# noamzilo/sed-crnn

Measured on AMD Instinct MI355X. Metric: mel-frames/sec training throughput (seq=256, mel=40), higher is better.
Workload: dtype f32; 1 GPU; BASELINE config 2: mono (B=128,256,40,1) per GPU, 3xConv3x3(128)+BN+ReLU+pool(1,2)+dropout0.5, BiGRU 2x128, Linear(256,1), BCEWithLogits, Adam lr 1e-3; full fit step (fwd+loss+bwd+allreduce+Adam); global_batch=128, seq_len=256, n_mels=40, parallelism=single

## Files before the change

### sed_crnn_amd/build.py

```python
import os
import subprocess
import sys
from concurrent.futures import ThreadPoolExecutor

HERE = os.path.dirname(os.path.abspath(__file__))
CSRC = os.path.join(HERE, "csrc")
OBJ = os.path.join(CSRC, "_obj")
LIB = os.path.join(HERE, "libsedcrnn.so")
SOURCES = ["api.cpp", "conv.hip", "conv_bf16.hip", "wino.hip", "conv1.hip", "bnpool.hip", "gemm.hip", "gru.hip", "misc.hip", "logmel.hip", "gcc.hip", "tdoa.hip", "doa.hip", "beam.hip", "mvdr.hip", "pcen.hip", "resample.hip", "data.hip", "detect.hip", "tune.hip", "stream.hip", "net.hip"]
FLAGS = ["--offload-arch=gfx950", "-O3", "-fPIC", "-std=c++17", "-Wall", "-Wno-unused-function"]
EXTRA_FLAGS = {"logmel.hip": ["-fno-slp-vectorize", "-Rpass-analysis=kernel-resource-usage"],
               "gcc.hip": ["-fno-slp-vectorize", "-Rpass-analysis=kernel-resource-usage"],
               "tdoa.hip": ["-fno-slp-vectorize", "-Rpass-analysis=kernel-resource-usage"],
               "doa.hip": ["-fno-slp-vectorize", "-Rpass-analysis=kernel-resource-usage"],
               "beam.hip": ["-fno-slp-vectorize", "-Rpass-analysis=kernel-resource-usage"],
               "mvdr.hip": ["-fno-slp-vectorize", "-Rpass-analysis=kernel-resource-usage"],
               "pcen.hip": ["-Rpass-analysis=kernel-resource-usage"],
               "conv.hip": ["-Rpass-analysis=kernel-resource-usage"],
               "wino.hip": ["-Rpass-analysis=kernel-resource-usage"],
               "conv_bf16.hip": ["-Rpass-analysis=kernel-resource-usage"],
               "gemm.hip": ["-Rpass-analysis=kernel-resource-usage"]}
NO_SPILL_KERNELS = {"conv.hip": ("conv3x3_mfma_fwd2_k", "conv3x3_mfma_fwd_bf16x3_k")}
NO_SCRATCH_KERNELS = {"wino.hip": ("conv3x3_wino_k",),
                      "conv_bf16.hip": ("conv3x3_bf16_eval_k", "gemm_bf16_nt_k"),
                      "logmel.hip": ("logmel_fft_k",),
                      "gcc.hip": ("gcc_phat_k",),
                      "tdoa.hip": ("tdoa_accum_k", "tdoa_finish_k"),
                      "doa.hip": ("doa_steer_k",),
                      "beam.hip": ("beam_sum_k", "beam_spans_k"),
                      "mvdr.hip": ("mvdr_cov_k", "mvdr_weights_k", "mvdr_apply_k", "mvdr_ring_cov_k", "mvdr_ring_apply_k"),
                      "pcen.hip": ("pcen_pass_k", "pcen_carry_k"),
                      "gemm.hip": ("gemm_f32_k",)}


def _hipcc():
    for c in (os.environ.get("HIPCC"), "/opt/rocm/bin/hipcc", "hipcc"):
        if c and (os.path.isabs(c) and os.path.exists(c) or not os.path.isabs(c)):
            return c
    raise RuntimeError("hipcc not found")


def _stale(target, deps):
    if not os.path.exists(target):
        return True
    t = os.path.getmtime(target)
    return any(os.path.getmtime(d) > t for d in deps)


def check_no_spill(remarks, kernels, allow_agprs=False):
    import re
    bad, seen, cur = [], set(), None
    for line in remarks.splitlines():
        m = re.search(r"remark: Function Name: (\S+)", line)
        if m:
            cur = next((k for k in kernels if k in m.group(1)), None)
            if cur:
                seen.add(cur)
            continue
        if cur:
            m = re.search(r"remark:\s+(ScratchSize \[bytes/lane\]|SGPRs Spill|VGPRs Spill|AGPRs): (\d+)", line)
            if m and int(m.group(2)) != 0 and not m.group(1).startswith("SGPRs") and not (allow_agprs and m.group(1) == "AGPRs"):
                bad.append(f"{cur}: {m.group(1)} = {m.group(2)}")
    bad += [f"{k}: no resource-usage remark found (kernel renamed? update NO_SPILL_KERNELS)" for k in kernels if k not in seen]
    return bad

# ... 53 lines not shown
```

### sed_crnn_amd/csrc/conv1.hip

```cpp
#include "common.h"

#define C1_TT 4
#define C1_MAXBLOCKS 2048

template <int CIN>
struct C1W { f32x4 w[9 * CIN]; f32x4 b; };

template <int CIN>
__device__ __forceinline__ void c1_load_w(C1W<CIN>& W, const float* __restrict__ wp, const float* __restrict__ bias,
                                          int Cout, int cg) {
#pragma unroll
    for (int tap = 0; tap < 9; ++tap)
#pragma unroll
        for (int ci = 0; ci < CIN; ++ci)
#pragma unroll
            for (int k = 0; k < 4; ++k) W.w[tap * CIN + ci][k] = wp[((size_t)tap * Cout + cg * 4 + k) * CIN + ci];
    W.b = bias ? *(const f32x4*)(bias + cg * 4) : (f32x4){0, 0, 0, 0};
}

template <int CIN>
__device__ __forceinline__ f32x4 c1_conv(const C1W<CIN>& W, const float* __restrict__ halo, int tl, int f, int F2) {
    f32x4 acc = W.b;
#pragma unroll
    for (int kh = 0; kh < 3; ++kh)
#pragma unroll
        for (int kw = 0; kw < 3; ++kw) {
            const float* hp = halo + ((tl + kw) * F2 + f + kh) * CIN;
#pragma unroll
            for (int ci = 0; ci < CIN; ++ci) acc += hp[ci] * W.w[(kh * 3 + kw) * CIN + ci];
        }
    return acc;
}

template <int CIN>
__device__ __forceinline__ void c1_conv2(const C1W<CIN>& W, const float* __restrict__ halo, int tl, int f, int F2,
                                         f32x4& v0, f32x4& v1) {
    float hv[4][3][CIN];
#pragma unroll
    for (int kw = 0; kw < 4; ++kw)
#pragma unroll
        for (int kh = 0; kh < 3; ++kh) {
            const float* hp = halo + ((tl + kw) * F2 + f + kh) * CIN;
#pragma unroll
            for (int ci = 0; ci < CIN; ++ci) hv[kw][kh][ci] = hp[ci];
        }
    v0 = W.b;
    v1 = W.b;
#pragma unroll
    for (int kh = 0; kh < 3; ++kh)
#pragma unroll
        for (int kw = 0; kw < 3; ++kw)
#pragma unroll
            for (int ci = 0; ci < CIN; ++ci) {
                v0 += hv[kw][kh][ci] * W.w[(kh * 3 + kw) * CIN + ci];
                v1 += hv[kw + 1][kh][ci] * W.w[(kh * 3 + kw) * CIN + ci];
            }
}

template <int CIN>
__device__ __forceinline__ void c1_stage(float* halo, const float* __restrict__ x, int b, int t0, int F, int T) {
    const int F2 = F + 2;
    const int n = (C1_TT + 2) * F2 * CIN;
    for (int i = threadIdx.x; i < n; i += 256) {
        int tt = i % (C1_TT + 2), ff = (i / (C1_TT + 2)) % F2, ci = i / ((C1_TT + 2) * F2);
        int t = t0 + tt - 1, f = ff - 1;
        float v = 0.f;
        if (t >= 0 && t < T && f >= 0 && f < F) v = x[(((size_t)b * CIN + ci) * F + f) * T + t];
        halo[(tt * F2 + ff) * CIN + ci] = v;
    }
}

template <int CIN, int MODE, bool P12>
__global__ __launch_bounds__(256) void conv1_fused_k(
    const float* __restrict__ x, const float* __restrict__ wp, const float* __restrict__ bias,
    const float* __restrict__ scale, const float* __restrict__ shift, const float* __restrict__ mean,
    const float* __restrict__ rstd, const float* __restrict__ sum_g, const float* __restrict__ sum_gx,
    const float* __restrict__ dout, float* __restrict__ out, float* __restrict__ partials,
    int B, int F, int T, int C, int pf, int pt, float drop_p, uint64_t seed, const uint64_t* __restrict__ seed_dev) {
    if (seed_dev) seed += seed_dev[0] * 0x9E3779B97F4A7C15ull;
    extern __shared__ __attribute__((aligned(16))) float smem[];
    if (P12) { pf = 1; pt = 2; }
    const int F2 = F + 2;
    float* halo = smem;
    const int tid = threadIdx.x;
    const int C4 = C >> 2, nslots = 256 / C4;
    const int cg = tid % C4, slot = tid / C4;
    const bool active = slot < nslots;
    const int tblocks = (T + C1_TT - 1) / C1_TT, ntiles = B * tblocks;
    const int Tp = T / pt, Fp = F / pf;
    const float inv_keep = drop_p > 0.f ? 1.f / (1.f - drop_p) : 1.f;
    const float invN = 1.f / ((float)B * (float)T * (float)F);

    C1W<CIN> W;
    if (active) c1_load_w<CIN>(W, wp, bias, C, cg);
    f32x4 sc = {0, 0, 0, 0}, sh = sc, mu = sc, rs = sc, sg = sc, sgx = sc;
    if (active && MODE >= 1) {
        sc = *(const f32x4*)(scale + cg * 4);
        sh = *(const f32x4*)(shift + cg * 4);
        if (MODE >= 2 && MODE != 4) { mu = *(const f32x4*)(mean + cg * 4); rs = *(const f32x4*)(rstd + cg * 4); }
        if (MODE == 3) { sg = *(const f32x4*)(sum_g + cg * 4) * invN; sgx = *(const f32x4*)(sum_gx + cg * 4) * invN; }
    }
    f32x4 a1 = {0, 0, 0, 0}, a2 = {0, 0, 0, 0};
    f32x4 dw[MODE == 3 ? 9 * CIN : 1];
    if (MODE == 3) {
#pragma unroll
        for (int k = 0; k < 9 * CIN; ++k) dw[k] = (f32x4){0, 0, 0, 0};
    }

    for (int tile = blockIdx.x; tile < ntiles; tile += gridDim.x) {
        const int b = tile / tblocks, t0 = (tile - b * tblocks) * C1_TT;
        __syncthreads();
        c1_stage<CIN>(halo, x, b, t0, F, T);
        __syncthreads();
        if (!active) continue;
        if (MODE == 0) {
            for (int p = slot; p < C1_TT * F; p += nslots) {
                int tl = p / F, f = p - tl * F;
                if (t0 + tl >= T) break;
                f32x4 v = c1_conv<CIN>(W, halo, tl, f, F2);
                a1 += v;
                a2 += v * v;
            }
        } else {
            const int tpn = C1_TT / pt;
            for (int op = slot; op < tpn * Fp; op += nslots) {
                int tpl = op / Fp, fp = op - tpl * Fp;
                int tp = t0 / pt + tpl;
                if (tp >= Tp) break;
                size_t oi = ((((size_t)b * Tp + tp) * Fp + fp) * C4 + cg) * 4;
                f32x4 vw[2];
                if (P12 && MODE >= 1) c1_conv2<CIN>(W, halo, tpl * 2, fp, F2, vw[0], vw[1]);
                if (MODE == 1) {
                    f32x4 m = {0, 0, 0, 0};
#pragma unroll
                    for (int df = 0; df < (P12 ? 1 : pf); ++df)
#pragma unroll
                        for (int dt = 0; dt < (P12 ? 2 : pt); ++dt) {
                            f32x4 z = (P12 ? vw[dt] : c1_conv<CIN>(W, halo, tpl * pt + dt, fp * pf + df, F2)) * sc + sh;
#pragma unroll
                            for (int k = 0; k < 4; ++k) m[k] = fmaxf(m[k], z[k]);
                        }
                    if (P12 && partials) {
                        const f32x4 z0 = vw[0] * sc + sh, z1 = vw[1] * sc + sh;
                        unsigned bt = 0;
#pragma unroll
                        for (int k = 0; k < 4; ++k) bt |= (z1[k] > z0[k] ? 1u : 0u) << k;
                        reinterpret_cast<unsigned char*>(partials)[oi >> 2] = (unsigned char)bt;
                    }
                    if (drop_p > 0.f) {
#pragma unroll
                        for (int k = 0; k < 4; ++k) m[k] *= sed_drop_mult(seed, oi + k, drop_p, inv_keep);
                    }
                    *(f32x4*)(out + oi) = m;
                } else {
                    f32x4 g = {0, 0, 0, 0};
                    if (MODE != 4) {
                        g = *(const f32x4*)(dout + oi);
                        if (drop_p > 0.f) {
#pragma unroll
                            for (int k = 0; k < 4; ++k) g[k] *= sed_drop_mult(seed, oi + k, drop_p, inv_keep);
                        }
                    }
                    f32x4 best = {-INFINITY, -INFINITY, -INFINITY, -INFINITY}, bx = {0, 0, 0, 0};
                    int bidx[4] = {0, 0, 0, 0};
                    int widx = 0;
#pragma unroll
                    for (int df = 0; df < (P12 ? 1 : pf); ++df)
#pragma unroll
                        for (int dt = 0; dt < (P12 ? 2 : pt); ++dt, ++widx) {
                            f32x4 v = P12 ? vw[dt] : c1_conv<CIN>(W, halo, tpl * pt + dt, fp * pf + df, F2);
                            f32x4 z = v * sc + sh;
#pragma unroll
                            for (int k = 0; k < 4; ++k)
                                if (z[k] > best[k]) { best[k] = z[k]; bx[k] = (v[k] - mu[k]) * rs[k]; bidx[k] = widx; }
                        }
                    if (MODE == 4) {
                        uchar4 code;
                        code.x = best[0] > 0.f ? (unsigned char)(1 + bidx[0]) : 0;
                        code.y = best[1] > 0.f ? (unsigned char)(1 + bidx[1]) : 0;
                        code.z = best[2] > 0.f ? (unsigned char)(1 + bidx[2]) : 0;
                        code.w = best[3] > 0.f ? (unsigned char)(1 + bidx[3]) : 0;
                        *(uchar4*)(reinterpret_cast<unsigned char*>(out) + oi) = code;
                        continue;
                    }
#pragma unroll
                    for (int k = 0; k < 4; ++k)
                        if (!(best[k] > 0.f)) g[k] = 0.f;
                    if (MODE == 2) {
                        a1 += g;
                        a2 += g * bx;
                    } else {
                        widx = 0;
#pragma unroll
                        for (int df = 0; df < (P12 ? 1 : pf); ++df)
#pragma unroll
                            for (int dt = 0; dt < (P12 ? 2 : pt); ++dt, ++widx) {
                                const int tl = tpl * pt + dt, f = fp * pf + df;
                                f32x4 v = P12 ? vw[dt] : c1_conv<CIN>(W, halo, tl, f, F2);
                                f32x4 o;
#pragma unroll
                                for (int k = 0; k < 4; ++k) {
                                    float xh = (v[k] - mu[k]) * rs[k];
                                    float gk = (bidx[k] == widx) ? g[k] : 0.f;
                                    o[k] = sc[k] * (gk - sg[k] - xh * sgx[k]);
                                    a2[k] += gk * xh;
                                }
                                a1 += o;
#pragma unroll
                                for (int kh = 0; kh < 3; ++kh)
#pragma unroll
                                    for (int kw = 0; kw < 3; ++kw) {
                                        const float* hp = halo + ((tl + kw) * F2 + f + kh) * CIN;
#pragma unroll
                                        for (int ci = 0; ci < CIN; ++ci) dw[(kh * 3 + kw) * CIN + ci] += hp[ci] * o;
                                    }
                            }
                    }
                }
            }
        }
    }
    if (MODE == 1 || MODE == 4) return;
    constexpr int NV = (MODE == 3) ? 2 + 9 * CIN : 2;
    constexpr int NVC = (MODE == 3) ? 5 : 2;
    float* red = smem;
#pragma unroll
    for (int v0 = 0; v0 < NV; v0 += NVC) {
        __syncthreads();
        if (active) {
#pragma unroll
            for (int j = 0; j < NVC; ++j) {
                const int v = v0 + j;
                if (v < NV) {
                    f32x4 val = (v == 0) ? a1 : ((MODE == 3 && v <= 9 * CIN) ? dw[(v - 1) < 9 * CIN ? (v - 1) : 0] : a2);
                    *(f32x4*)(red + (slot * NVC + j) * C + cg * 4) = val;
                }
            }
        }
        __syncthreads();
        const int nv = (NV - v0 < NVC) ? NV - v0 : NVC;
        for (int i = tid; i < nv * C; i += 256) {
            int j = i / C, c = i - j * C;
            float a = 0.f;
            for (int s = 0; s < nslots; ++s) a += red[(s * NVC + j) * C + c];
            partials[(size_t)blockIdx.x * NV * C + (size_t)(v0 + j) * C + c] = a;
// ... 542 lines not shown
            const double w2 = (double)wp[((size_t)(k2 / Cin) * C + co) * Cin + (k2 % Cin)];
            wg += w2 * gram[k <= k2 ? c1_gidx(k, k2, NK) : c1_gidx(k2, k, NK)];
        }
        const double s1 = gram[k];
        const double val = sc * (sv[1 + k] - sg * s1 - sgx * rs * (b * s1 + wg - mu * s1));
        const int tap = k / Cin, ci = k - tap * Cin;
        dw[((size_t)co * Cin + ci) * 9 + tap] = (float)val;
    }
    if (lane == 63) {
        const double sum_y = count * b + ws1;
        db[co] = (float)(sc * (sv[0] - count * sg - sgx * rs * (sum_y - count * mu)));
        if (dgamma && (own || (gamma && beta && gamma[co] == 0.f && beta[co] > 0.f))) dgamma[co] = (float)sgx_sum;
    }
}

static size_t c1_lds(int Cin, int F, int C, int mode) {
    size_t halo = (size_t)(C1_TT + 2) * (F + 2) * Cin * sizeof(float);
    size_t nv = mode == 3 ? 5 : 2;
    size_t red = (size_t)256 * 4 * nv * sizeof(float);
    return halo > red ? halo : red;
}

static int c1_shape_ok(int Cin, int F, int T, int C, int pool_f, int pool_t, int max_cin);
extern "C" int sed_conv1_fused_supported(int Cin, int F, int T, int C, int pool_f, int pool_t) {
    return c1_shape_ok(Cin, F, T, C, pool_f, pool_t, 2);
}
static int c1_shape_ok(int Cin, int F, int T, int C, int pool_f, int pool_t, int max_cin) {
    if (Cin < 1 || Cin > max_cin || C < 4 || F < 1 || T < 1 || C % 4 != 0 || C / 4 > 256 || (256 % (C / 4)) != 0) return 0;
    if (pool_t < 1 || pool_f < 1 || C1_TT % pool_t != 0 || T % C1_TT != 0 || F % pool_f != 0 || T % pool_t != 0) return 0;
    if (c1_lds(Cin, F, C, 3) > 150 * 1024) return 0;
    return 1;
}

extern "C" int sed_conv1_fused_rows(int B, int T) {
    long n = (long)B * ((T + C1_TT - 1) / C1_TT);
    return (int)(n < C1_MAXBLOCKS ? n : C1_MAXBLOCKS);
}

template <int MODE>
static int c1_launch(const float* x, const float* wp, const float* bias, const float* scale, const float* shift,
                     const float* mean, const float* rstd, const float* sum_g, const float* sum_gx, const float* dout,
                     float* out, float* partials, int B, int Cin, int F, int T, int C, int pf, int pt, float drop_p,
                     uint64_t seed, const uint64_t* seed_dev, hipStream_t s) {
    size_t lds = c1_lds(Cin, F, C, MODE);
    int grid = sed_conv1_fused_rows(B, T);
    const bool p12 = (pf == 1 && pt == 2);
#define C1_LAUNCH(CIN_, P12_)                                                                                          \
    do {                                                                                                               \
        if (lds > 48 * 1024)                                                                                           \
            (void)hipFuncSetAttribute((const void*)conv1_fused_k<CIN_, MODE, P12_>, hipFuncAttributeMaxDynamicSharedMemorySize, (int)lds); \
        conv1_fused_k<CIN_, MODE, P12_><<<grid, 256, lds, s>>>(x, wp, bias, scale, shift, mean, rstd, sum_g, sum_gx, dout, out, \
                                                              partials, B, F, T, C, pf, pt, drop_p, seed, seed_dev);  \
    } while (0)
    if (Cin == 1) { if (p12) C1_LAUNCH(1, true); else C1_LAUNCH(1, false); }
    else if (Cin == 2) { if (p12) C1_LAUNCH(2, true); else C1_LAUNCH(2, false); }
    else if ((MODE == 1 || MODE == 4) && p12) {
        if (Cin == 3) C1_LAUNCH(3, true);
        else C1_LAUNCH(4, true);
    } else {
        sed_set_error("conv1: %d input channels are supported by the forward pass with the (1,2) pool only", Cin);
        return SED_EUNSUPPORTED;
    }
#undef C1_LAUNCH
    return 0;
}

#define C1_CHECK(who)                                                                                             \
    SED_REQUIRE(sed_conv1_fused_supported(Cin, F, T, C, pf, pt), who ": shape Cin=%d F=%d T=%d C=%d pool=(%d,%d) is not " \
                "supported by the fused first block", Cin, F, T, C, pf, pt)

extern "C" size_t sed_conv1_stats_workspace_bytes(int B, int Cin, int T) {
    const int nk = 9 * Cin;
    if (Cin > 2) {
        const int nt = (nk + 1 + 15) / 16, np = nt * (nt + 1) / 2;
        return (size_t)C1_MM_BLOCKS * np * 256 * sizeof(float) + (size_t)(nk + nk * (nk + 1) / 2) * sizeof(double);
    }
    return (size_t)256 * (nk + nk * (nk + 1) / 2) * sizeof(float);
}

static int conv1_stats_impl(const float* x, const float* wp, const float* bias, float* stat_partials, void* workspace,
                            int B, int Cin, int F, int T, int C, double* gram_out, const Conv1BnOut& bn, void* stream);

extern "C" int sed_conv1_stats(const float* x, const float* wp, const float* bias, float* stat_partials, void* workspace,
                               int B, int Cin, int F, int T, int C, double* gram_out, void* stream) {
    return conv1_stats_impl(x, wp, bias, stat_partials, workspace, B, Cin, F, T, C, gram_out, Conv1BnOut{}, stream);
}

int sed_internal_conv1_stats_bn(const float* x, const float* wp, const float* bias, float* stat_partials, void* workspace,
                                int B, int Cin, int F, int T, int C, double* gram_out, const float* gamma, const float* beta,
                                float* running_mean, float* running_var, float momentum, float eps,
                                float* mean, float* rstd, float* scale, float* shift, void* stream) {
    SED_REQUIRE(Cin >= 1 && Cin <= 2, "conv1_stats_bn: Cin=%d (the merged finalisation exists for 1 or 2 input channels)", Cin);
    SED_REQUIRE(gamma && beta && mean && rstd && scale && shift, "conv1_stats_bn: null pointer");
    return conv1_stats_impl(x, wp, bias, stat_partials, workspace, B, Cin, F, T, C, gram_out,
                            Conv1BnOut{gamma, beta, running_mean, running_var, momentum, eps, mean, rstd, scale, shift}, stream);
}
// ... 26 lines not shown
        SED_LAUNCH_CHECK("conv1_moments");
        return 0;
    }
    int grid =(B * ((T + C1_GT - 1) / C1_GT) + C1_GR - 1) / C1_GR;
    if (grid > 256) grid = 256;
    const int nk = 9 * Cin, ng = nk + nk * (nk + 1) / 2;
    size_t lds = (size_t)C1_GR * (C1_GT + 2) * (F + 2) * Cin * sizeof(float), red = (size_t)ng * 4 * sizeof(float);
    SED_REQUIRE(lds <= 150 * 1024, "conv1_stats: F=%d Cin=%d needs %zu B of LDS", F, Cin, lds);
    if (red > lds) lds = red;
    const double count = (double)B * T * F;
    if (lds > 48 * 1024) {
        (void)hipFuncSetAttribute((const void*)conv1_gram_k<1>, hipFuncAttributeMaxDynamicSharedMemorySize, (int)lds);
        (void)hipFuncSetAttribute((const void*)conv1_gram_k<2>, hipFuncAttributeMaxDynamicSharedMemorySize, (int)lds);
    }
    if (Cin == 1) {
        conv1_gram_k<1><<<grid, 256, lds, s>>>(x, (float*)workspace, B, F, T);
        SED_LAUNCH_CHECK("conv1_gram");
        conv1_gram_finalize_k<1><<<1, 256, 0, s>>>((const float*)workspace, grid, wp, bias, count, C, stat_partials, gram_out, bn);
    } else {
        conv1_gram_k<2><<<grid, 256, lds, s>>>(x, (float*)workspace, B, F, T);
        SED_LAUNCH_CHECK("conv1_gram");
        conv1_gram_finalize_k<2><<<1, 256, 0, s>>>((const float*)workspace, grid, wp, bias, count, C, stat_partials, gram_out, bn);
    }
    SED_LAUNCH_CHECK("conv1_gram_finalize");
    return 0;
}

extern "C" int sed_conv1_bn_relu_pool_drop_fwd(const float* x, const float* wp, const float* bias, const float* scale,
                                               const float* shift, float* out, int B, int Cin, int F, int T, int C,
                                               int pf, int pt, float drop_p, uint64_t seed, const uint64_t* seed_dev,
                                               unsigned char* argmax_bits, void* stream) {
    SED_REQUIRE(x && wp && scale && shift && out, "conv1_fwd: null pointer");
    SED_REQUIRE(drop_p >= 0.f && drop_p < 1.f, "conv1_fwd: drop_p=%f out of [0,1)", drop_p);
    SED_REQUIRE(c1_shape_ok(Cin, F, T, C, pf, pt, (pf == 1 && pt == 2) ? 4 : 2), "conv1_fwd: shape Cin=%d F=%d T=%d C=%d pool=(%d,%d) is not "
                "supported by the fused first block", Cin, F, T, C, pf, pt);
    hipStream_t s = as_stream(stream);
    SedProfScope prof(SED_K_BN_FWD, s, 4.0 * B * C * (double)(T / pt) * (F / pf));
    SED_REQUIRE(!argmax_bits || (pf == 1 && pt == 2), "conv1_fwd: arg-max bits exist for the (1,2) pool only");
    SED_TRY(c1_launch<1>(x, wp, bias, scale, shift, nullptr, nullptr, nullptr, nullptr, nullptr, out, reinterpret_cast<float*>(argmax_bits), B, Cin, F, T, C, pf, pt, drop_p, seed, seed_dev, s));
    SED_LAUNCH_CHECK("conv1_fwd");
    return 0;
}

extern "C" int sed_conv1_route(const float* x, const float* wp, const float* bias, const float* scale, const float* shift,
                               unsigned char* route, int B, int Cin, int F, int T, int C, int pf, int pt, void* stream) {
    SED_REQUIRE(x && wp && scale && shift && route, "conv1_route: null pointer");
    SED_REQUIRE(c1_shape_ok(Cin, F, T, C, pf, pt, (pf == 1 && pt == 2) ? 4 : 2), "conv1_route: shape Cin=%d F=%d T=%d C=%d pool=(%d,%d) is not "
                "supported by the fused first block", Cin, F, T, C, pf, pt);
    SED_REQUIRE(pf * pt <= 254, "conv1_route: a %dx%d window does not fit the one-byte code", pf, pt);
    SED_TRY(c1_launch<4>(x, wp, bias, scale, shift, nullptr, nullptr, nullptr, nullptr, nullptr, reinterpret_cast<float*>(route), nullptr,
                         B, Cin, F, T, C, pf, pt, 0.f, 0, nullptr, as_stream(stream)));
    SED_LAUNCH_CHECK("conv1_route");
    return 0;
}

extern "C" int sed_conv1_bwd_reduce(const float* x, const float* wp, const float* bias, const float* dout,
                                    const float* scale, const float* shift, const float* mean, const float* rstd,
                                    float* partials, int B, int Cin, int F, int T, int C, int pf, int pt, float drop_p,
                                    uint64_t seed, const uint64_t* seed_dev, void* stream) {
    SED_REQUIRE(x && wp && dout && scale && shift && mean && rstd && partials, "conv1_bwd_reduce: null pointer");
    C1_CHECK("conv1_bwd_reduce");
    hipStream_t s = as_stream(stream);
    SedProfScope prof(SED_K_BN_BWD_REDUCE, s, 4.0 * B * C * (double)(T / pt) * (F / pf));
    c1_launch<2>(x, wp, bias, scale, shift, mean, rstd, nullptr, nullptr, dout, nullptr, partials, B, Cin, F, T, C, pf, pt, drop_p, seed, seed_dev, s);
    SED_LAUNCH_CHECK("conv1_bwd_reduce");
    return 0;
}

extern "C" size_t sed_conv1_bwd_apply_workspace_bytes(int B, int Cin, int T, int C) {
    return (size_t)sed_conv1_fused_rows(B, T) * (2 + 9 * Cin) * C * sizeof(float);
}

extern "C" int sed_conv1_bwd_apply_wgrad(const float* x, const float* wp, const float* bias, const float* dout,
                                         const float* scale, const float* shift, const float* mean, const float* rstd,
                                         const float* sum_g, const float* sum_gx, float* dw_oihw, float* dbias,
                                         void* workspace, int B, int Cin, int F, int T, int C, int pf, int pt,
                                         float drop_p, uint64_t seed, const uint64_t* seed_dev,
                                         const float* gamma, const float* beta, float* dgamma, void* stream) {
    SED_REQUIRE(x && wp && dout && scale && shift && mean && rstd && sum_g && sum_gx && dw_oihw && dbias && workspace,
                "conv1_bwd_apply_wgrad: null pointer");
    C1_CHECK("conv1_bwd_apply_wgrad");
    hipStream_t s = as_stream(stream);
    SedProfScope prof(SED_K_BN_BWD_APPLY, s, 4.0 * B * C * (double)(T / pt) * (F / pf));
    c1_launch<3>(x, wp, bias, scale, shift, mean, rstd, sum_g, sum_gx, dout, nullptr, (float*)workspace, B, Cin, F, T, C, pf, pt, drop_p, seed, seed_dev, s);
    SED_LAUNCH_CHECK("conv1_bwd_apply_wgrad");
    int rows = sed_conv1_fused_rows(B, T), n = (2 + 9 * Cin) * C;
    conv1_wgrad_reduce_k<<<cdiv(n, 8), 256, 0, s>>>((const float*)workspace, rows, Cin, C, dw_oihw, dbias, gamma, beta, dgamma);
    SED_LAUNCH_CHECK("conv1_wgrad_reduce");
    return 0;
}

extern "C" int sed_conv1_rgrad_supported(int Cin, int F, int T, int C, int pf, int pt) {
    return pf == 1 && pt == 2 && c1_shape_ok(Cin, F, T, C, pf, pt, 4);
}
// ... 67 lines not shown
```

### sed_crnn_amd/csrc/gru.hip

```cpp
#include "common.h"

static inline int gru_bt(int H, int B) {
    int bt = B >= 512 ? 4 : (B >= 256 ? 2 : 1);
    if (H >= 128 && bt > 2) bt = 2;
    return bt;
}

__global__ void gru_pack_whh_t_k(const float* __restrict__ w0, const float* __restrict__ w1,
                                 float* __restrict__ wt, int H) {
    int i = blockIdx.x * blockDim.x + threadIdx.x;
    int n = 3 * H * H;
    if (i >= 2 * n) return;
    int dir = i / n, e = i - dir * n;
    int g = e / H, k = e - g * H;
    const float* w = dir ? w1 : w0;
    wt[(size_t)dir * n + (size_t)k * 3 * H + g] = w[e];
}

constexpr int gru_nt(int hreg) { return hreg > 0 ? ((3 * hreg + 63) / 64) * 64 : 1024; }

__device__ __forceinline__ float gru_dot4(float w0, float w1, float w2, float w3, const f32x4& h) {
    return fmaf(w3, h[3], fmaf(w2, h[2], fmaf(w0, h[0], w1 * h[1])));
}

template <int HREG, int GRU_BT, int HTOT = HREG, int HLDS = 0>
__global__ __launch_bounds__(gru_nt(HTOT)) void gru_seq_fwd_k(
    const float* __restrict__ gi, const float* __restrict__ wt, const float* __restrict__ bhh0,
    const float* __restrict__ bhh1, float* __restrict__ out, float* __restrict__ saved, int B, int T, int H) {
    extern __shared__ __attribute__((aligned(16))) float smem[];
    float* h_s = smem;
    float* gh_s = smem + GRU_BT * H;
    float* w_l = smem + GRU_BT * 4 * H;
    const int g = threadIdx.x;
    const int dir = blockIdx.y, b0 = blockIdx.x * GRU_BT;
    const int H3 = 3 * H;
    const float* wtd = wt + (size_t)dir * H3 * H;
    const float* bhh = dir ? bhh1 : bhh0;
    const bool row = g < H3;
    const bool gate = g < H;
    constexpr bool HYB = HTOT != HREG && HREG > 0;

    float wreg[HREG > 0 ? HREG : 1];
    if (HREG > 0 && row) {
#pragma unroll
        for (int k = 0; k < HREG; ++k) wreg[k] = wtd[(size_t)k * H3 + g];
    }
    if (HYB && row) {
        for (int j = 0; j < HLDS; ++j) w_l[j * H3 + g] = wtd[(size_t)(HREG + j) * H3 + g];
    }
    const float bias = row ? bhh[g] : 0.f;
    for (int i = g; i < GRU_BT * H; i += blockDim.x) h_s[i] = 0.f;
    __syncthreads();

    float gr[GRU_BT], gz[GRU_BT], gn[GRU_BT], nr[GRU_BT], nz[GRU_BT], nn[GRU_BT], mr[GRU_BT], mz[GRU_BT], mn[GRU_BT];
    auto fetch_gi = [&](int s, float* a, float* bq, float* c) {
        const int tt = dir ? (T - 1 - s) : s;
#pragma unroll
        for (int b = 0; b < GRU_BT; ++b) {
            int bg = b0 + b;
            if (gate && bg < B && s < T) {
                const float* p = gi + (((size_t)bg * T + tt) * 2 + dir) * H3;
                a[b] = p[g]; bq[b] = p[H + g]; c[b] = p[2 * H + g];
            } else { a[b] = bq[b] = c[b] = 0.f; }
        }
    };
    fetch_gi(0, gr, gz, gn);
    fetch_gi(1, nr, nz, nn);
    for (int s = 0; s < T; ++s) {
        const int tt = dir ? (T - 1 - s) : s;
        fetch_gi(s + 2, mr, mz, mn);
        if (row) {
            float acc[GRU_BT];
#pragma unroll
            for (int b = 0; b < GRU_BT; ++b) acc[b] = bias;
            if (HREG > 0) {
#pragma unroll
                for (int k = 0; k < HREG; k += 4) {
#pragma unroll
                    for (int b = 0; b < GRU_BT; ++b) {
                        f32x4 hv = *(const f32x4*)(h_s + b * H + k);
                        acc[b] += gru_dot4(wreg[k], wreg[k + 1], wreg[k + 2], wreg[k + 3], hv);
                    }
                }
            }
// ... 229 lines not shown
    else if (v.bt == 2) KERNEL<HR, 2><<<grid, nt, lds, s>>>(__VA_ARGS__);                     \
    else KERNEL<HR, 4><<<grid, nt, lds, s>>>(__VA_ARGS__)
#define GRU_DISPATCH(KERNEL, ...)                                                             \
    if (v.hlds > 0) {                                                                         \
        KERNEL<GRU_HRX, 1, 256, GRU_HL><<<grid, nt, lds + (size_t)GRU_HL * 768 * sizeof(float), s>>>(__VA_ARGS__); \
    } else switch (v.hreg) {                                                                  \
        case 8: GRU_BT3(8, KERNEL, __VA_ARGS__); break;                                       \
        case 16: GRU_BT3(16, KERNEL, __VA_ARGS__); break;                                     \
        case 32: GRU_BT3(32, KERNEL, __VA_ARGS__); break;                                     \
        case 64: GRU_BT3(64, KERNEL, __VA_ARGS__); break;                                     \
        case 128:                                                                             \
            if (v.bt == 1) KERNEL<128, 1><<<grid, nt, lds, s>>>(__VA_ARGS__);                 \
            else KERNEL<128, 2><<<grid, nt, lds, s>>>(__VA_ARGS__);                           \
            break;                                                                            \
        default: GRU_BT3(0, KERNEL, __VA_ARGS__); break;                                      \
    }

static int gru_pack_whh(const float* const* whh, float* wt, int H, hipStream_t s) {
    int n = 2 * 3 * H * H;
    gru_pack_whh_t_k<<<cdiv(n, 256), 256, 0, s>>>(whh[0], whh[1], wt, H);
    SED_LAUNCH_CHECK("gru_pack_whh_t");
    return 0;
}

int sed_internal_gru_seq_fwd_packed(const float* gi, const float* wt, const float* const* bhh, float* out,
                                    float* saved, int B, int T, int H, void* stream) {
    SED_REQUIRE(gi && wt && bhh && out && bhh[0] && bhh[1], "gru_seq_fwd: null pointer");
    SED_REQUIRE(B > 0 && T > 0 && H > 0 && H % 4 == 0 && 3 * H <= 1024, "gru_seq_fwd: H=%d must be a multiple of 4 and <= 341", H);
    hipStream_t s = as_stream(stream);
    const GruVariant v = gru_variant(H, B, GRU_HR_FWD);
    dim3 grid(cdiv(B, v.bt), 2);
    int nt = gru_threads(H);
    size_t lds = (size_t)v.bt * 4 * H * sizeof(float);
    SedProfScope prof(SED_K_GRU_FWD, s, 2.0 * 2 * B * (double)T * 3 * H * H);
    if (v.hlds > 0)
        (void)hipFuncSetAttribute((const void*)gru_seq_fwd_k<GRU_HR_FWD, 1, 256, GRU_HL>, hipFuncAttributeMaxDynamicSharedMemorySize, 160 * 1024);
#define GRU_HRX GRU_HR_FWD
    GRU_DISPATCH(gru_seq_fwd_k, gi, wt, bhh[0], bhh[1], out, saved, B, T, H);
#undef GRU_HRX
    SED_LAUNCH_CHECK("gru_seq_fwd");
    return 0;
}

extern "C" int sed_gru_seq_fwd(const float* gi, const float* const* whh, const float* const* bhh, float* out,
                               float* saved, void* workspace, int B, int T, int H, void* stream) {
    SED_REQUIRE(gi && whh && bhh && out && workspace && whh[0] && whh[1] && bhh[0] && bhh[1], "gru_seq_fwd: null pointer");
    SED_REQUIRE(B > 0 && T > 0 && H > 0 && H % 4 == 0 && 3 * H <= 1024, "gru_seq_fwd: H=%d must be a multiple of 4 and <= 341", H);
    SED_TRY(gru_pack_whh(whh, (float*)workspace, H, as_stream(stream)));
    return sed_internal_gru_seq_fwd_packed(gi, (const float*)workspace, bhh, out, saved, B, T, H, stream);
}

extern "C" size_t sed_gru_seq_bwd_workspace_bytes(int B, int H) { return (size_t)cdiv(B, gru_bt(H, B)) * 2 * 4 * H * sizeof(float); }

int sed_internal_gru_seq_bwd_partials(const float* dout, const float* saved, const float* const* whh, float* dgi,
                                      float* dgh, float* bpart, int B, int T, int H, void* stream) {
    SED_REQUIRE(dout && saved && whh && whh[0] && whh[1] && dgi && dgh, "gru_seq_bwd: null pointer");
    SED_REQUIRE(B > 0 && T > 0 && H > 0 && H % 4 == 0 && 3 * H <= 1024, "gru_seq_bwd: H=%d must be a multiple of 4 and <= 341", H);
    hipStream_t s = as_stream(stream);
    const GruVariant v = gru_variant(H, B, GRU_HR);
    dim3 grid(cdiv(B, v.bt), 2);
    int nt = gru_threads(H);
    size_t lds = (size_t)v.bt * 6 * H * sizeof(float);
    SedProfScope prof(SED_K_GRU_BWD, s, 2.0 * 2 * B * (double)T * 3 * H * H);
    if (v.hlds > 0)
        (void)hipFuncSetAttribute((const void*)gru_seq_bwd_k<GRU_HR, 1, 256, GRU_HL>, hipFuncAttributeMaxDynamicSharedMemorySize, 160 * 1024);
#define GRU_HRX GRU_HR
// ... 25 lines not shown
```

Baseline: 6.025 million mel-frames/s.

## Warp-specialize GRU forward with LDS ring prefetch and strength-reduce conv1 indexing

The GRU forward kernel, when all recurrent weights fit in registers, now splits waves into gate, load and row roles. Loader waves prefetch input-gate values two steps ahead into a three-slot LDS ring, so global loads stay off the recurrent critical path. The fused first conv kernel replaces per-iteration divisions and 64-bit index math with incremental pointer and offset updates, and uses 32-bit dropout hashing unless the tensor is very large. It also adds occupancy hints via launch bounds and a no-spill build check. The cost is extra LDS for the ring and some added complexity in synchronisation and role dispatch.

```diff
diff --git a/sed_crnn_amd/build.py b/sed_crnn_amd/build.py
--- a/sed_crnn_amd/build.py
+++ b/sed_crnn_amd/build.py
@@ -16,6 +16,7 @@
                "beam.hip": ["-fno-slp-vectorize", "-Rpass-analysis=kernel-resource-usage"],
                "mvdr.hip": ["-fno-slp-vectorize", "-Rpass-analysis=kernel-resource-usage"],
                "pcen.hip": ["-Rpass-analysis=kernel-resource-usage"],
+               "conv1.hip": ["-Rpass-analysis=kernel-resource-usage"],
                "conv.hip": ["-Rpass-analysis=kernel-resource-usage"],
                "wino.hip": ["-Rpass-analysis=kernel-resource-usage"],
                "conv_bf16.hip": ["-Rpass-analysis=kernel-resource-usage"],
@@ -30,7 +31,8 @@
                       "beam.hip": ("beam_sum_k", "beam_spans_k"),
                       "mvdr.hip": ("mvdr_cov_k", "mvdr_weights_k", "mvdr_apply_k", "mvdr_ring_cov_k", "mvdr_ring_apply_k"),
                       "pcen.hip": ("pcen_pass_k", "pcen_carry_k"),
-                      "gemm.hip": ("gemm_f32_k",)}
+                      "gemm.hip": ("gemm_f32_k",),
+                      "conv1.hip": ("conv1_fused_k",)}
 
 
 def _hipcc():
diff --git a/sed_crnn_amd/csrc/conv1.hip b/sed_crnn_amd/csrc/conv1.hip
--- a/sed_crnn_amd/csrc/conv1.hip
+++ b/sed_crnn_amd/csrc/conv1.hip
@@ -19,13 +19,13 @@
 }
 
 template <int CIN>
-__device__ __forceinline__ f32x4 c1_conv(const C1W<CIN>& W, const float* __restrict__ halo, int tl, int f, int F2) {
+__device__ __forceinline__ f32x4 c1_conv(const C1W<CIN>& W, const float* __restrict__ hb, int F2) {
     f32x4 acc = W.b;
 #pragma unroll
     for (int kh = 0; kh < 3; ++kh)
 #pragma unroll
         for (int kw = 0; kw < 3; ++kw) {
-            const float* hp = halo + ((tl + kw) * F2 + f + kh) * CIN;
+            const float* hp = hb + (kw * F2 + kh) * CIN;
 #pragma unroll
             for (int ci = 0; ci < CIN; ++ci) acc += hp[ci] * W.w[(kh * 3 + kw) * CIN + ci];
         }
@@ -33,14 +33,13 @@
 }
 
 template <int CIN>
-__device__ __forceinline__ void c1_conv2(const C1W<CIN>& W, const float* __restrict__ halo, int tl, int f, int F2,
-                                         f32x4& v0, f32x4& v1) {
+__device__ __forceinline__ void c1_conv2(const C1W<CIN>& W, const float* __restrict__ hb, int F2, f32x4& v0, f32x4& v1) {
     float hv[4][3][CIN];
 #pragma unroll
     for (int kw = 0; kw < 4; ++kw)
 #pragma unroll
         for (int kh = 0; kh < 3; ++kh) {
-            const float* hp = halo + ((tl + kw) * F2 + f + kh) * CIN;
+            const float* hp = hb + (kw * F2 + kh) * CIN;
 #pragma unroll
             for (int ci = 0; ci < CIN; ++ci) hv[kw][kh][ci] = hp[ci];
         }
@@ -70,8 +69,14 @@
     }
 }
 
-template <int CIN, int MODE, bool P12>
-__global__ __launch_bounds__(256) void conv1_fused_k(
+constexpr int c1_waves(int cin, int mode, bool p12) {
+    if (mode == 1 || mode == 4) return cin == 1 ? 5 : (cin == 2 ? ((mode == 1 && p12) ? 3 : 4) : 2);
+    if (mode == 2) return cin == 1 ? 4 : (cin == 2 ? 3 : 2);
+    return cin <= 2 ? 2 : 1;
+}
+
+template <int CIN, int MODE, bool P12, bool IDX64 = false>
+__global__ __launch_bounds__(256, c1_waves(CIN, MODE, P12)) void conv1_fused_k(
     const float* __restrict__ x, const float* __restrict__ wp, const float* __restrict__ bias,
     const float* __restrict__ scale, const float* __restrict__ shift, const float* __restrict__ mean,
     const float* __restrict__ rstd, const float* __restrict__ sum_g, const float* __restrict__ sum_gx,
@@ -107,36 +112,60 @@
         for (int k = 0; k < 9 * CIN; ++k) dw[k] = (f32x4){0, 0, 0, 0};
     }
 
-    for (int tile = blockIdx.x; tile < ntiles; tile += gridDim.x) {
-        const int b = tile / tblocks, t0 = (tile - b * tblocks) * C1_TT;
+    const int pos_w = (MODE == 0) ? F : Fp;
+    const int row_h = (MODE == 0) ? F2 * CIN : pt * F2 * CIN;
+    const int pos_h = (MODE == 0) ? CIN : pf * CIN;
+    const int q0 = nslots / pos_w, dfp = nslots - q0 * pos_w;
+    const int tpl0 = slot / pos_w, fp0 = slot - tpl0 * pos_w;
+    const int dhb = q0 * row_h + dfp * pos_h, whb = row_h - pos_w * pos_h;
+    const unsigned doff = (unsigned)nslots * C4 * 4;
+    const int qb = gridDim.x / tblocks, qt = gridDim.x - qb * tblocks;
+    int b = blockIdx.x / tblocks, tb = blockIdx.x - b * tblocks;
+
+    for (int tile = blockIdx.x; tile < ntiles; tile += gridDim.x, b += qb, tb += qt) {
+        if (tb >= tblocks) { tb -= tblocks; ++b; }
+        const int t0 = tb * C1_TT;
         __syncthreads();
         c1_stage<CIN>(halo, x, b, t0, F, T);
         __syncthreads();
         if (!active) continue;
         if (MODE == 0) {
+            int tl = tpl0, f = fp0;
+            const float* hb = halo + tpl0 * row_h + fp0 * pos_h;
             for (int p = slot; p < C1_TT * F; p += nslots) {
-                int tl = p / F, f = p - tl * F;
                 if (t0 + tl >= T) break;
-                f32x4 v = c1_conv<CIN>(W, halo, tl, f, F2);
+                f32x4 v = c1_conv<CIN>(W, hb, F2);
                 a1 += v;
                 a2 += v * v;
+                tl += q0; f += dfp; hb += dhb;
+                if (f >= F) { f -= F; ++tl; hb += whb; }
             }
         } else {
             const int tpn = C1_TT / pt;
-            for (int op = slot; op < tpn * Fp; op += nslots) {
-                int tpl = op / Fp, fp = op - tpl * Fp;
-                int tp = t0 / pt + tpl;
-                if (tp >= Tp) break;
-                size_t oi = ((((size_t)b * Tp + tp) * Fp + fp) * C4 + cg) * 4;
+            const int tp0 = t0 / pt;
+            const size_t tbase = ((size_t)b * Tp + tp0) * Fp * C;
+            const uint32_t tb_lo = (uint32_t)tbase;
+            auto keep_mult = [&](unsigned offk) {
+                return sed_drop_mult(seed, IDX64 ? (uint64_t)tbase + offk : (uint64_t)(uint32_t)(tb_lo + offk), drop_p, inv_keep);
+            };
+            int tpl = tpl0, fp = fp0;
+            const float* hb = halo + tpl0 * row_h + fp0 * pos_h;
+            unsigned off = (unsigned)(slot * C4 + cg) * 4;
+            for (int op = slot; op < tpn * Fp; op += nslots, off += doff) {
+                if (tp0 + tpl >= Tp) break;
+                const float* hw = hb;
+                tpl += q0; fp += dfp; hb += dhb;
+                if (fp >= Fp) { fp -= Fp; ++tpl; hb += whb; }
+                const unsigned boff = off * 4u;
                 f32x4 vw[2];
-                if (P12 && MODE >= 1) c1_conv2<CIN>(W, halo, tpl * 2, fp, F2, vw[0], vw[1]);
+                if (P12 && MODE >= 1) c1_conv2<CIN>(W, hw, F2, vw[0], vw[1]);
                 if (MODE == 1) {
                     f32x4 m = {0, 0, 0, 0};
 #pragma unroll
                     for (int df = 0; df < (P12 ? 1 : pf); ++df)
 #pragma unroll
                         for (int dt = 0; dt < (P12 ? 2 : pt); ++dt) {
-                            f32x4 z = (P12 ? vw[dt] : c1_conv<CIN>(W, halo, tpl * pt + dt, fp * pf + df, F2)) * sc + sh;
+                            f32x4 z = (P12 ? vw[dt] : c1_conv<CIN>(W, hw + (dt * F2 + df) * CIN, F2)) * sc + sh;
 #pragma unroll
                             for (int k = 0; k < 4; ++k) m[k] = fmaxf(m[k], z[k]);
                         }
@@ -145,20 +174,22 @@
                         unsigned bt = 0;
 #pragma unroll
                         for (int k = 0; k < 4; ++k) bt |= (z1[k] > z0[k] ? 1u : 0u) << k;
-                        reinterpret_cast<unsigned char*>(partials)[oi >> 2] = (unsigned char)bt;
+                        (reinterpret_cast<unsigned char*>(partials) + (tbase >> 2))[off >> 2] = (unsigned char)bt;
                     }
                     if (drop_p > 0.f) {
 #pragma unroll
-                        for (int k = 0; k < 4; ++k) m[k] *= sed_drop_mult(seed, oi + k, drop_p, inv_keep);
+                        for (int k = 0; k < 4; ++k)
+                            m[k] *= keep_mult(off + k);
                     }
-                    *(f32x4*)(out + oi) = m;
+                    *(f32x4*)((char*)(out + tbase) + boff) = m;
                 } else {
                     f32x4 g = {0, 0, 0, 0};
                     if (MODE != 4) {
-                        g = *(const f32x4*)(dout + oi);
+                        g = *(const f32x4*)((const char*)(dout + tbase) + boff);
                         if (drop_p > 0.f) {
 #pragma unroll
-                            for (int k = 0; k < 4; ++k) g[k] *= sed_drop_mult(seed, oi + k, drop_p, inv_keep);
+                            for (int k = 0; k < 4; ++k)
+                                g[k] *= keep_mult(off + k);
                         }
                     }
                     f32x4 best = {-INFINITY, -INFINITY, -INFINITY, -INFINITY}, bx = {0, 0, 0, 0};
@@ -168,7 +199,7 @@
                     for (int df = 0; df < (P12 ? 1 : pf); ++df)
 #pragma unroll
                         for (int dt = 0; dt < (P12 ? 2 : pt); ++dt, ++widx) {
-                            f32x4 v = P12 ? vw[dt] : c1_conv<CIN>(W, halo, tpl * pt + dt, fp * pf + df, F2);
+                            f32x4 v = P12 ? vw[dt] : c1_conv<CIN>(W, hw + (dt * F2 + df) * CIN, F2);
                             f32x4 z = v * sc + sh;
 #pragma unroll
                             for (int k = 0; k < 4; ++k)
@@ -180,7 +211,7 @@
                         code.y = best[1] > 0.f ? (unsigned char)(1 + bidx[1]) : 0;
                         code.z = best[2] > 0.f ? (unsigned char)(1 + bidx[2]) : 0;
                         code.w = best[3] > 0.f ? (unsigned char)(1 + bidx[3]) : 0;
-                        *(uchar4*)(reinterpret_cast<unsigned char*>(out) + oi) = code;
+                        *(uchar4*)(reinterpret_cast<unsigned char*>(out) + tbase + off) = code;
                         continue;
                     }
 #pragma unroll
@@ -195,8 +226,8 @@
                         for (int df = 0; df < (P12 ? 1 : pf); ++df)
 #pragma unroll
                             for (int dt = 0; dt < (P12 ? 2 : pt); ++dt, ++widx) {
-                                const int tl = tpl * pt + dt, f = fp * pf + df;
-                                f32x4 v = P12 ? vw[dt] : c1_conv<CIN>(W, halo, tl, f, F2);
+                                const float* he = hw + (dt * F2 + df) * CIN;
+                                f32x4 v = P12 ? vw[dt] : c1_conv<CIN>(W, he, F2);
                                 f32x4 o;
 #pragma unroll
                                 for (int k = 0; k < 4; ++k) {
@@ -210,7 +241,7 @@
                                 for (int kh = 0; kh < 3; ++kh)
 #pragma unroll
                                     for (int kw = 0; kw < 3; ++kw) {
-                                        const float* hp = halo + ((tl + kw) * F2 + f + kh) * CIN;
+                                        const float* hp = he + (kw * F2 + kh) * CIN;
 #pragma unroll
                                         for (int ci = 0; ci < CIN; ++ci) dw[(kh * 3 + kw) * CIN + ci] += hp[ci] * o;
                                     }
@@ -819,6 +850,11 @@
     return 1;
 }
 
+static int c1_pass_shape_ok(int Cin, int F, int T, int C, int pool_f, int pool_t, int max_cin) {
+    if (T < 1 || pool_t < 1 || T % pool_t != 0) return 0;
+    return c1_shape_ok(Cin, F, (T + C1_TT - 1) / C1_TT * C1_TT, C, pool_f, pool_t, max_cin);
+}
+
 extern "C" int sed_conv1_fused_rows(int B, int T) {
     long n = (long)B * ((T + C1_TT - 1) / C1_TT);
     return (int)(n < C1_MAXBLOCKS ? n : C1_MAXBLOCKS);
@@ -832,12 +868,17 @@
     size_t lds = c1_lds(Cin, F, C, MODE);
     int grid = sed_conv1_fused_rows(B, T);
     const bool p12 = (pf == 1 && pt == 2);
+    const bool idx64 = MODE != 4 && drop_p > 0.f && (size_t)B * (T / pt) * (F / pf) * C > 0xFFFFFFFFull;
+#define C1_LAUNCH_(CIN_, P12_, I64_)                                                                                   \
+    do {                                                                                                               \
+        if (lds > 48 * 1024)                                                                                           \
+            (void)hipFuncSetAttribute((const void*)conv1_fused_k<CIN_, MODE, P12_, I64_>, hipFuncAttributeMaxDynamicSharedMemorySize, (int)lds); \
+        conv1_fused_k<CIN_, MODE, P12_, I64_><<<grid, 256, lds, s>>>(x, wp, bias, scale, shift, mean, rstd, sum_g, sum_gx, dout, out, \
+                                                                    partials, B, F, T, C, pf, pt, drop_p, seed, seed_dev); \
+    } while (0)
 #define C1_LAUNCH(CIN_, P12_)                                                                                          \
     do {                                                                                                               \
-        if (lds > 48 * 1024)                                                                                           \
-            (void)hipFuncSetAttribute((const void*)conv1_fused_k<CIN_, MODE, P12_>, hipFuncAttributeMaxDynamicSharedMemorySize, (int)lds); \
-        conv1_fused_k<CIN_, MODE, P12_><<<grid, 256, lds, s>>>(x, wp, bias, scale, shift, mean, rstd, sum_g, sum_gx, dout, out, \
-                                                              partials, B, F, T, C, pf, pt, drop_p, seed, seed_dev);  \
+        if (MODE != 4 && idx64) C1_LAUNCH_(CIN_, P12_, (MODE != 4)); else C1_LAUNCH_(CIN_, P12_, false);               \
     } while (0)
     if (Cin == 1) { if (p12) C1_LAUNCH(1, true); else C1_LAUNCH(1, false); }
     else if (Cin == 2) { if (p12) C1_LAUNCH(2, true); else C1_LAUNCH(2, false); }
@@ -849,6 +890,7 @@
         return SED_EUNSUPPORTED;
     }
 #undef C1_LAUNCH
+#undef C1_LAUNCH_
     return 0;
 }
 
@@ -941,7 +983,7 @@
                                                unsigned char* argmax_bits, void* stream) {
     SED_REQUIRE(x && wp && scale && shift && out, "conv1_fwd: null pointer");
     SED_REQUIRE(drop_p >= 0.f && drop_p < 1.f, "conv1_fwd: drop_p=%f out of [0,1)", drop_p);
-    SED_REQUIRE(c1_shape_ok(Cin, F, T, C, pf, pt, (pf == 1 && pt == 2) ? 4 : 2), "conv1_fwd: shape Cin=%d F=%d T=%d C=%d pool=(%d,%d) is not "
+    SED_REQUIRE(c1_pass_shape_ok(Cin, F, T, C, pf, pt, (pf == 1 && pt == 2) ? 4 : 2), "conv1_fwd: shape Cin=%d F=%d T=%d C=%d pool=(%d,%d) is not "
                 "supported by the fused first block", Cin, F, T, C, pf, pt);
     hipStream_t s = as_stream(stream);
     SedProfScope prof(SED_K_BN_FWD, s, 4.0 * B * C * (double)(T / pt) * (F / pf));
@@ -954,7 +996,7 @@
 extern "C" int sed_conv1_route(const float* x, const float* wp, const float* bias, const float* scale, const float* shift,
                                unsigned char* route, int B, int Cin, int F, int T, int C, int pf, int pt, void* stream) {
     SED_REQUIRE(x && wp && scale && shift && route, "conv1_route: null pointer");
-    SED_REQUIRE(c1_shape_ok(Cin, F, T, C, pf, pt, (pf == 1 && pt == 2) ? 4 : 2), "conv1_route: shape Cin=%d F=%d T=%d C=%d pool=(%d,%d) is not "
+    SED_REQUIRE(c1_pass_shape_ok(Cin, F, T, C, pf, pt, (pf == 1 && pt == 2) ? 4 : 2), "conv1_route: shape Cin=%d F=%d T=%d C=%d pool=(%d,%d) is not "
                 "supported by the fused first block", Cin, F, T, C, pf, pt);
     SED_REQUIRE(pf * pt <= 254, "conv1_route: a %dx%d window does not fit the one-byte code", pf, pt);
     SED_TRY(c1_launch<4>(x, wp, bias, scale, shift, nullptr, nullptr, nullptr, nullptr, nullptr, reinterpret_cast<float*>(route), nullptr,
@@ -968,7 +1010,8 @@
                                     float* partials, int B, int Cin, int F, int T, int C, int pf, int pt, float drop_p,
                                     uint64_t seed, const uint64_t* seed_dev, void* stream) {
     SED_REQUIRE(x && wp && dout && scale && shift && mean && rstd && partials, "conv1_bwd_reduce: null pointer");
-    C1_CHECK("conv1_bwd_reduce");
+    SED_REQUIRE(c1_pass_shape_ok(Cin, F, T, C, pf, pt, 2), "conv1_bwd_reduce: shape Cin=%d F=%d T=%d C=%d pool=(%d,%d) is not "
+                "supported by the fused first block", Cin, F, T, C, pf, pt);
     hipStream_t s = as_stream(stream);
     SedProfScope prof(SED_K_BN_BWD_REDUCE, s, 4.0 * B * C * (double)(T / pt) * (F / pf));
     c1_launch<2>(x, wp, bias, scale, shift, mean, rstd, nullptr, nullptr, dout, nullptr, partials, B, Cin, F, T, C, pf, pt, drop_p, seed, seed_dev, s);
diff --git a/sed_crnn_amd/csrc/gru.hip b/sed_crnn_amd/csrc/gru.hip
--- a/sed_crnn_amd/csrc/gru.hip
+++ b/sed_crnn_amd/csrc/gru.hip
@@ -23,6 +23,102 @@
     return fmaf(w3, h[3], fmaf(w2, h[2], fmaf(w0, h[0], w1 * h[1])));
 }
 
+enum { GRU_GATE = 0, GRU_LOAD = 1, GRU_ROW = 2, GRU_ALL = 3 };
+
+template <int HREG, int GRU_BT, int ROLE>
+__device__ __forceinline__ void gru_fwd_ring(const float* __restrict__ gi, float* __restrict__ out, float* __restrict__ saved,
+                                             float* h_s, float* gh_s, float* ring, const float (&wreg)[HREG], const float bias,
+                                             const int g, const int li, const int dir, const int b0, const int B, const int T, const int H) {
+    constexpr bool GATES = ROLE == GRU_GATE || ROLE == GRU_ALL, LOADS = ROLE == GRU_LOAD || ROLE == GRU_ALL;
+    const int H3 = 3 * H;
+    const bool row = g < H3, gate = g < H;
+    const bool lane = li < H;
+    const int lic = lane ? li : 0;
+    float xa[GRU_BT][3], xb[GRU_BT][3];
+    auto issue = [&](int s, float (*q)[3]) {
+        const int sc = s < T ? s : T - 1;
+        const int tt = dir ? (T - 1 - sc) : sc;
+#pragma unroll
+        for (int b = 0; b < GRU_BT; ++b) {
+            const int bg = b0 + b < B ? b0 + b : B - 1;
+            const float* p = gi + (((size_t)bg * T + tt) * 2 + dir) * H3 + lic;
+            q[b][0] = p[0]; q[b][1] = p[H]; q[b][2] = p[2 * H];
+        }
+    };
+    auto commit = [&](float (*q)[3], int slot) {
+        float* r = ring + slot * (GRU_BT * H3);
+#pragma unroll
+        for (int b = 0; b < GRU_BT; ++b) {
+            const bool in = b0 + b < B;
+            const float v0 = in ? q[b][0] : 0.f, v1 = in ? q[b][1] : 0.f, v2 = in ? q[b][2] : 0.f;
+            if (lane) { r[b * H3 + li] = v0; r[b * H3 + H + li] = v1; r[b * H3 + 2 * H + li] = v2; }
+        }
+    };
+    int rd = 0;
+    auto step = [&](int s, float (*nw)[3], float (*ld)[3]) {
+        const int tt = dir ? (T - 1 - s) : s;
+        if (LOADS) issue(s + 2, nw);
+        if (row) {
+            float acc[GRU_BT];
+#pragma unroll
+            for (int b = 0; b < GRU_BT; ++b) acc[b] = bias;
+#pragma unroll
+            for (int k = 0; k < HREG; k += 4) {
+#pragma unroll
+                for (int b = 0; b < GRU_BT; ++b) {
+                    f32x4 hv = *(const f32x4*)(h_s + b * H + k);
+                    acc[b] += gru_dot4(wreg[k], wreg[k + 1], wreg[k + 2], wreg[k + 3], hv);
+                }
+            }
+#pragma unroll
+            for (int b = 0; b < GRU_BT; ++b) gh_s[b * H3 + g] = acc[b];
+        }
+        __syncthreads();
+        if (GATES && gate) {
+            const float* rg = ring + rd * (GRU_BT * H3);
+            float gr[GRU_BT], gz[GRU_BT], gn[GRU_BT];
+#pragma unroll
+            for (int b = 0; b < GRU_BT; ++b) {
+                int bg = b0 + b;
+                gr[b] = rg[b * H3 + g]; gz[b] = rg[b * H3 + H + g]; gn[b] = rg[b * H3 + 2 * H + g];
+                float ghr = gh_s[b * H3 + g], ghz = gh_s[b * H3 + H + g], ghn = gh_s[b * H3 + 2 * H + g];
+                float hp = h_s[b * H + g];
+                float r = __fdividef(1.f, 1.f + __expf(-(gr[b] + ghr)));
+                float z = __fdividef(1.f, 1.f + __expf(-(gz[b] + ghz)));
+                float a = gn[b] + r * ghn;
+                float e2 = __expf(-2.f * fabsf(a));
+                float n = copysignf(__fdividef(1.f - e2, 1.f + e2), a);
+                float hn = (1.f - z) * n + z * hp;
+                h_s[b * H + g] = hn;
+                if (bg < B) {
+                    out[((size_t)bg * T + tt) * 2 * H + dir * H + g] = hn;
+                    if (saved) {
+                        float* sp = saved + ((((size_t)bg * T + tt) * 2 + dir) * 5) * H + g;
+                        sp[0] = r; sp[H] = z; sp[2 * H] = n; sp[3 * H] = ghn; sp[4 * H] = hp;
+                    }
+                }
+            }
+        }
+        rd = rd == 2 ? 0 : rd + 1;
+        if (LOADS) commit(ld, rd);
+        __syncthreads();
+    };
+    if (LOADS) { issue(0, xa); issue(1, xb); commit(xa, 0); }
+    __syncthreads();
+    int s = 0;
+    for (; s + 1 < T; s += 2) {
+        step(s, xa, xb);
+        step(s + 1, xb, xa);
+    }
+    if (s < T) step(s, xa, xb);
+    if (LOADS) {
+#pragma unroll
+        for (int b = 0; b < GRU_BT; ++b)
+#pragma unroll
+            for (int e = 0; e < 3; ++e) asm volatile("" : : "v"(xa[b][e]), "v"(xb[b][e]));
+    }
+}
+
 template <int HREG, int GRU_BT, int HTOT = HREG, int HLDS = 0>
 __global__ __launch_bounds__(gru_nt(HTOT)) void gru_seq_fwd_k(
     const float* __restrict__ gi, const float* __restrict__ wt, const float* __restrict__ bhh0,
@@ -31,6 +127,7 @@
     float* h_s = smem;
     float* gh_s = smem + GRU_BT * H;
     float* w_l = smem + GRU_BT * 4 * H;
+    float* ring = smem + GRU_BT * 4 * H;
     const int g = threadIdx.x;
     const int dir = blockIdx.y, b0 = blockIdx.x * GRU_BT;
     const int H3 = 3 * H;
@@ -50,6 +147,23 @@
     }
     const float bias = row ? bhh[g] : 0.f;
     for (int i = g; i < GRU_BT * H; i += blockDim.x) h_s[i] = 0.f;
+    if constexpr (HREG > 0 && !HYB) {
+        constexpr int NW = gru_nt(HTOT) / 64, GW = (HTOT + 63) / 64;
+#pragma unroll
+        for (int k = 0; k < HREG; ++k) asm volatile("" : "+v"(wreg[k]));
+        float bias_r = bias;
+        asm volatile("" : "+v"(bias_r));
+        if constexpr (NW >= 2 * GW) {
+            const int wave = __builtin_amdgcn_readfirstlane(g >> 6);
+            if (wave < GW) gru_fwd_ring<HREG, GRU_BT, GRU_GATE>(gi, out, saved, h_s, gh_s, ring, wreg, bias_r, g, 0, dir, b0, B, T, H);
+            else if (NW == 2 * GW || wave < 2 * GW)
+                gru_fwd_ring<HREG, GRU_BT, GRU_LOAD>(gi, out, saved, h_s, gh_s, ring, wreg, bias_r, g, g - 64 * GW, dir, b0, B, T, H);
+            else gru_fwd_ring<HREG, GRU_BT, GRU_ROW>(gi, out, saved, h_s, gh_s, ring, wreg, bias_r, g, 0, dir, b0, B, T, H);
+        } else {
+            gru_fwd_ring<HREG, GRU_BT, GRU_ALL>(gi, out, saved, h_s, gh_s, ring, wreg, bias_r, g, g, dir, b0, B, T, H);
+        }
+        return;
+    }
     __syncthreads();
 
     float gr[GRU_BT], gz[GRU_BT], gn[GRU_BT], nr[GRU_BT], nz[GRU_BT], nn[GRU_BT], mr[GRU_BT], mz[GRU_BT], mn[GRU_BT];
@@ -345,6 +459,7 @@
     dim3 grid(cdiv(B, v.bt), 2);
     int nt = gru_threads(H);
     size_t lds = (size_t)v.bt * 4 * H * sizeof(float);
+    if (v.hreg == H) lds += (size_t)3 * v.bt * 3 * H * sizeof(float);
     SedProfScope prof(SED_K_GRU_FWD, s, 2.0 * 2 * B * (double)T * 3 * H * H);
     if (v.hlds > 0)
         (void)hipFuncSetAttribute((const void*)gru_seq_fwd_k<GRU_HR_FWD, 1, 256, GRU_HL>, hipFuncAttributeMaxDynamicSharedMemorySize, 160 * 1024);
```

Result: no change. 6.067 million mel-frames/s (median of 6 runs) (+0.7%).
